# umr-lops/xsarsea

Measured on AMD Instinct MI355X. Metric: Mpixels/s wind inversion (CMOD5.N, 20k x 20k sigma0), higher is better.
Workload: dtype f64; 1 GPU; CMOD5.N mono-VV inversion (the metric's raster), 20000x20000 float32 sigma0/incidence + complex64 ancillary, default LUT 501x499x181 (90319 candidates/pixel), complex64 out, algo=pruned, sigma0 -> dB fused on the device; lines=20000, samples=20000, lines_rank0=20000, parallelism=row tiles x1

## Files before the change

xsarsea_amd/csrc/xsw_band.hpp:

```cpp
#pragma once
#include "xsw_device.hpp"

namespace xsw {

#ifndef XSW_BAND_MAX
#define XSW_BAND_MAX 64
#endif
#ifndef XSW_BAND_RAY_D
#define XSW_BAND_RAY_D 2
#endif
#ifndef XSW_LONG_RUN_MAX
#define XSW_LONG_RUN_MAX 128
#endif
#ifndef XSW_LONG_RUN_MAX_CUT
#define XSW_LONG_RUN_MAX_CUT 64
#endif
#ifndef XSW_SWEEP_MAX
#define XSW_SWEEP_MAX 128
#endif
#ifndef XSW_B2_HARD_AREA
#define XSW_B2_HARD_AREA 256
#endif
#ifndef XSW_BAND_SEEDED
#define XSW_BAND_SEEDED 1
// ... 5 lines not shown
#define XSW_BAND_WG_WAVES 4
#endif
#ifndef XSW_BAND_POOL
#define XSW_BAND_POOL 1
#endif
static_assert(XSW_BAND_WG_WAVES % 4 == 0 || !XSW_BAND_POOL, "pooled class counts are read as four bytes per word");
#ifndef XSW_BAND_WAVES
#define XSW_BAND_WAVES 8
#endif
#ifndef XSW_BAND_BATCH_S
#define XSW_BAND_BATCH_S 2
#endif
#ifndef XSW_BAND_BATCH
#define XSW_BAND_BATCH 4
#endif
#ifndef XSW_BAND_WAVES_CR
#define XSW_BAND_WAVES_CR 7
#endif
#ifndef XSW_BAND2_WAVES
#define XSW_BAND2_WAVES 4
#endif

struct BandSlot {
    double sn, thr_lo, thr_hi, ah, bh, m2;
    int inc_bin , rows , ipn ;
    int bin_hi ;
};

constexpr int kBandClasses = 11;
struct BandPool {
    alignas(4) unsigned char cnt[kBandClasses][XSW_BAND_WG_WAVES];
    unsigned short map[64 * XSW_BAND_WG_WAVES];
};
__device__ __forceinline__ int byte_sum4(unsigned x)
{
    x = (x & 0x00ff00ffu) + ((x >> 8) & 0x00ff00ffu);
    return (int)((x & 0xffffu) + (x >> 16));
}

struct BandRec {
    double s, ah, bh;
    float d;
    int inc_tail;
    int rows;
    int ipn;
    unsigned idx;
    int flags;
};
struct Band2Slot;
constexpr int kBand2SlotBytes = 56;
template <typename T, typename TO, bool CR>
// ... 41 lines not shown
            for (int e = 0; e < 2; ++e) {
                const int ip = gc + 2 * h + e;
                const int ra = (int)((wa[h] >> (e * 16)) & 0xffffu), rb = (int)((wb[h] >> (e * 16)) & 0xffffu);
                const float uh = e ? uhx * c4.z + uhy * c4.w : uhx * c4.x + uhy * c4.y;
                const int lo = max(w_lo, ra), hi = capped ? min(w_hi, rb - 1) : w_hi;
                const float t = vminf(vmaxf(uh, fmaf((float)lo, whs, wh0)), fmaf((float)max(hi, lo), whs, wh0));
                const float jw = fmaf(t, t - 2.0f * uh, m2) - XSW_BOUND_SLACK * (m2 + t * (t + 2.0f * fabsf(uh)));
                const bool live = gact && ip >= ip_lo && ip < ip_end && lo <= hi && !(jw > jub);
                first = (live && first == 0x7fff) ? ip : first;
                last = live ? ip : last;
            }
        }
    }
    return last >= 0 ? (unsigned)first | ((unsigned)last << 16) : 0x00007fffu;
}
__device__ __forceinline__ double ld_co(const char *__restrict__ base, unsigned off0, int row, unsigned rowB)
{
    return *(const double *)(base + (off0 + __umul24((unsigned)row, rowB)));
}

#ifndef XSW_CHORD_MRG
#define XSW_CHORD_MRG 2e-3
#endif
template <int S, int K, bool COUNT>
__device__ __forceinline__ void co_band_pass(const DevTables &L, double inv_dsig, int lane,
                                             const BandSlot *slots , int *res ,
                                             int first, int count , unsigned &cand,
                                             const unsigned short *map = nullptr )
{
    constexpr int sweep_max = XSW_BAND_MAX;
    const double inf = __builtin_inf();
    const int q = lane / S, sl = lane & (S - 1);
    const bool valid = q < count;
    const int owner = valid ? (map ? (int)map[first + q] : first + q) : lane;
    BandSlot B = slots[owner];
    if (!valid) { B.inc_bin = 0; B.rows = 0; B.ipn = 0; B.bin_hi = -1; }
    const int B_ip_lo = B.ipn & 0xffff, B_ncols = (int)((unsigned)B.ipn >> 16);
    const int w_lo = B.rows & 0xffff, w_hi = B.rows >> 16;
    const double thr_lo = B.thr_lo, thr_hi = B.thr_hi, sn = B.sn;
    const double wh0 = 0.5 * L.w0, whs = L.wstep_half;
    const char *__restrict__ base = (const char *)L.co;
    const unsigned rowB = (unsigned)L.phi_pad * 8u;
    const int i_inc = B.inc_bin & 0xffff;
    const unsigned slice0 = mul24_sv(rowB, mul24_sv((unsigned)L.n_w, (unsigned)i_inc));
    const unsigned short *__restrict__ inv_tab = L.inv_rows;
    const unsigned inv_rowB = (unsigned)L.phi_pad * 2u;
    const unsigned inv0 = mul24_sv(inv_rowB, (unsigned)(i_inc * XSW_INV_BINS) + ((unsigned)B.inc_bin >> 16));
    const unsigned inv1 = mul24_sv(inv_rowB, (unsigned)(i_inc * XSW_INV_BINS) + (unsigned)max(B.bin_hi, 0));
    double best = inf, second = inf;
    int brow = 0, bip = 0;
    unsigned ncand = 0;
    bool overflow = false;
    const int nchunks = S == 64 ? (__builtin_amdgcn_readfirstlane(B_ncols) + 64 * K - 1) / (64 * K) : 1;
#pragma unroll 1
    for (int ch = 0; ch < nchunks; ++ch) {
        bool act[K];
        int ip[K], r[K], nrow[K];
        unsigned off0[K];
        double U[K];
#pragma unroll
        for (int j = 0; j < K; ++j) {
            const int vcol = sl + S * j + S * K * ch;
            act[j] = valid && vcol < B_ncols;
            ip[j] = B_ip_lo + (act[j] ? vcol : 0);
            const unsigned ipB = (unsigned)ip[j] * 8u;
            const double2 cs = *(const double2 *)((const char *)L.csphi + 2u * ipB);
            U[j] = 2.0 * (B.ah * cs.x + B.bh * cs.y);
            off0[j] = slice0 + ipB;
        }
        int nmax = 0;
#pragma unroll
        for (int j = 0; j < K; ++j) {
            const unsigned o_first = inv0 + (unsigned)ip[j] * 2u, o_last = inv1 + (unsigned)ip[j] * 2u;
            const int ra = (int)*(const unsigned short *)((const char *)inv_tab + o_first);
            const int rb = (int)*(const unsigned short *)((const char *)inv_tab + o_last);
            r[j] = max(ra, w_lo);
            const int last = B.bin_hi >= 0 ? min(rb - 1, w_hi) : w_hi;
            nrow[j] = act[j] ? last - r[j] + 1 : 0;
            nmax = max(nmax, nrow[j]);
        }
#pragma unroll 1
        for (int t = 0; t < XSW_BAND_MAX; ++t) {
            unsigned long long left[K], any_left = 0ULL;
#pragma unroll
            for (int j = 0; j < K; ++j) { left[j] = ballot64(t < nrow[j]); any_left |= left[j]; }
            if (any_left == 0ULL) break;
#pragma unroll
            for (int j = 0; j < K; ++j) {
                if (left[j] == 0ULL) continue;
                const int rc = min(r[j] + t, w_hi);
                const double v = ld_co(base, off0[j], rc, rowB);
                const bool inb = t < nrow[j];
                const double wh = fma((double)rc, whs, wh0);
                const double dd = fma(v, inv_dsig, sn);
                double J = fma(dd, dd, wh * (wh - U[j]));
                J = __hiloint2double(inb ? __double2hiint(J) : 0x7FE00000, __double2loint(J));
                second = vmin(second, vmax(J, best));
                const bool lt = J < best;
                brow = lt ? rc : brow;
                if (K > 1 || S == 64) bip = lt ? ip[j] : bip;
                best = vmin(best, J);
                if (COUNT) ncand += inb ? 1u : 0u;
            }
        }
        const bool any = nmax > sweep_max;
        overflow = overflow || any;
        if (K == 1 && S != 64) bip = ip[0];
    }
    const int bflat = (int)__umul24((unsigned)brow, (unsigned)L.n_phi) + bip;
    const double gmin = S == 64 ? wave_min_d(best) : seg_min_d<S>(best);
    const double T = gmin + 1e-9 * (1.0 + fabs(gmin) + slots[owner].m2);
    const unsigned long long amb = ballot64(valid && (second <= T || overflow)), surv = ballot64(valid && best <= T);
    const unsigned long long segmask = S == 64 ? ~0ULL : (((1ULL << (S & 63)) - 1ULL) << ((q * S) & 63));
    const bool bad = (amb & segmask) != 0ULL || __popcll(surv & segmask) != 1 || !(gmin < 1e300);
    if (valid && ((!bad && best <= T) || (bad && sl == 0))) res[owner] = bad ? -1 : bflat;
    if (COUNT) {
        unsigned c = ncand;
        for (int off = 32; off > 0; off >>= 1) c += __shfl_xor(c, off);
        cand += c;
    }
}

__device__ __forceinline__ bool list_append(unsigned *__restrict__ count, unsigned *__restrict__ list, unsigned cap, bool flag, long long i, int lane)
{
    const unsigned long long um = __ballot(flag);
    if (!um) return false;
    unsigned base = 0;
    if (lane == 0) base = atomicAdd(count, (unsigned)__popcll(um));
    base = (unsigned)__builtin_amdgcn_readfirstlane((int)base);
    const unsigned at = base + __builtin_amdgcn_mbcnt_hi((unsigned)(um >> 32), __builtin_amdgcn_mbcnt_lo((unsigned)um, 0u));
    if (flag && at < cap) list[at] = (unsigned)i;
    return flag && at >= cap;
}
__device__ __forceinline__ void mask_mark(unsigned long long *__restrict__ mask, bool flag, long long i, long long strip, long long samples, int lane)
{
    const unsigned long long m = __ballot(flag);
    if (!m) return;
    if (strip >= 0) {
// ... 43 lines not shown
    if (A.list_b) drop_b = A.rec_b ? (unresolved && to_b) : list_append(A.list_b_count, A.list_b, A.list_b_cap, unresolved && to_b, i, lane);
    if (A.list_c) drop_c = list_append(A.list_c_count, A.list_c, A.list_c_cap, unresolved && to_c && !to_b, i, lane);
    const bool for_c = A.list_c != nullptr && to_c && !to_b && !drop_c;
    const bool drop_g = list_append(A.list_count, A.list, A.list_cap, unresolved && !to_b && !for_c, i, lane);
    if (A.mask_g) {
        if (A.list_b) mask_mark(A.mask_b, drop_b, i, strip, A.samples, lane);
        mask_mark(A.mask_g, drop_g, i, strip, A.samples, lane);
    }
    if (in) {
        if (!unresolved) {
            Pixel Q;
            Q.flags = flags;
            Q.a_re = nan; Q.a_im = nan;
            if (A.anc) {
                typename Cx<T>::type z = ((const typename Cx<T>::type *)A.anc)[i];
                Q.a_re = (double)z.x;
                Q.a_im = (double)z.y;
            }
            store_pixel<TO, CR>(L, A, i, Q, my_flat, my_icr);
        }
    }
}

template <typename T, typename TO, bool CR, bool COUNT, int ROLE = 0>
__device__ __forceinline__ void band_wave(const DevTables &L, const KArgs &A, long long i, bool in, int lane, BandSlot *__restrict__ slots,
                                          int *__restrict__ res_, bool strip_walk = false ,
                                          long long strip = -1 ,
                                          BandPool *__restrict__ pool = nullptr )
{
    const double nan = __builtin_nan("");
    int flags, my_flat = -1, my_icr = -1;
    unsigned cand = 0;
    constexpr int NC = kBandClasses;
    constexpr bool POOLED = XSW_BAND_POOL && ROLE != 2;
    constexpr int WG = XSW_BAND_WG_WAVES, PK = POOLED ? 64 * WG : 64;
    int pos = -1, myc = NC, first[NC] = {}, ncls[NC] = {};
    auto settle_queues = [&]() {
#pragma unroll
        for (int c = 0; c + 1 < NC; ++c) {
            const int np = 64 / (2 << (c >> 1)), npn = 64 / (2 << ((c + 1) >> 1));
            const int rem = ncls[c] % np;
            const int added = (ncls[c + 1] + rem + npn - 1) / npn - (ncls[c + 1] + npn - 1) / npn;
            if (rem > 0 && added == 0) { ncls[c] -= rem; ncls[c + 1] += rem; first[c + 1] -= rem; }
        }
#pragma unroll
        for (int c = 0; c < NC; ++c) {
            first[c] = __builtin_amdgcn_readfirstlane(first[c]);
            ncls[c] = __builtin_amdgcn_readfirstlane(ncls[c]);
        }
    };
    bool skip = false;
    {
        Pixel P;
        load_pixel<T, false>(L, A, i, in, P);
        flags = P.flags;
        if (CR && A.s_cr) {
            const T x = ((const T *)A.s_cr)[i];
            const T dr = A.dsig_cr ? ((const T *)A.dsig_cr)[i] : (T)0;
            if (x != x || dr != dr) flags |= F_CR_RAW_NAN;
        }
        const unsigned long long todo = __ballot((P.flags & F_NEED_CO) != 0);
        bool eligb = false;
        int ncols_p = 0;
        if (todo) {
            bool loose = false;
            CoWindow W = co_window_lanes<XSW_BAND_RAYS, XSW_BAND_RAY_D, XSW_BAND_SEEDED != 0>(L, P, A.inv_dsig_co, fabs(A.dsig_co), loose);
            int w_hi_e = W.w_hi;
            bool has_tail = false;
            if (L.tail_min) {
                const bool fin1 = (P.flags & F_NEED_CO) != 0 && (P.flags & F_CO_FINITE) != 0;
                const int mono1 = L.mono_rows[fin1 ? P.i_inc : 0];
                if (fin1 && W.w_hi >= mono1 && W.ip_hi >= W.ip_lo) {
                    const int len = W.ip_hi - W.ip_lo + 1, k = min(31 - __clz(len), XSW_TAIL_LEVELS);
                    const double *tk = L.tail_min + mul24_sv((unsigned)L.phi_pad, (unsigned)(P.i_inc * (XSW_TAIL_LEVELS + 1) + k));
                    const double lo = fmin(tk[W.ip_lo], tk[k < XSW_TAIL_LEVELS ? W.ip_hi - (1 << k) + 1 : W.ip_lo]);
                    if (P.s_co + W.band_d < lo) w_hi_e = mono1 - 1;
                    else if (ROLE != 0 && mono1 >= 1 && W.w_hi - mono1 + 1 <= A.tail_max) { has_tail = true; w_hi_e = mono1 - 1; }
                }
            }
            const int nrows_p = w_hi_e - W.w_lo + 1;
            ncols_p = W.ip_hi - W.ip_lo + 1;
            const bool need = (P.flags & F_NEED_CO) != 0 && (P.flags & F_CO_FINITE) != 0 && ncols_p >= 1 && (nrows_p >= 1 || has_tail);
            if (ROLE == 2 && strip_walk) skip = !need || !(w_hi_e < L.mono_rows[need ? P.i_inc : 0]);
            eligb = need && w_hi_e < L.mono_rows[need ? P.i_inc : 0];
            if (ROLE != 2 && need && !eligb) flags |= F_TO_C;
            if (COUNT) cand += (unsigned)__popcll(__ballot(eligb)) * (unsigned)(2 * (32 - __clz((L.n_w + 1) >> 1)) + (XSW_BAND_RAYS - 1) * 2 * XSW_RAY_SIDE_STEPS);
            double thr_lo = P.s_co - W.band_d, thr_hi = P.s_co + W.band_d;
            int bin = 0, bhi = XSW_INV_BINS;
            if (eligb) {
                const double *g = L.inv_grid + 3 * P.i_inc;
                const double t0 = g[0], width = g[1];
                bin = (int)fmin(fmax((thr_lo - t0) * g[2], 0.0), (double)(XSW_INV_BINS - 1));
                if (bin > 0 && fma((double)bin, width, t0) > thr_lo) --bin;
                if (bin > 0 && fma((double)bin, width, t0) > thr_lo) bin = 0;
// ... 70 lines not shown
                const unsigned long long m = __ballot(myc == c);
                const int rank = (int)__builtin_amdgcn_mbcnt_hi((unsigned)(m >> 32), __builtin_amdgcn_mbcnt_lo((unsigned)m, 0u));
                pos = myc == c ? base + rank : pos;
                first[c] = base;
                ncls[c] = __popcll(m);
                base += ncls[c];
            }
            if constexpr (!POOLED) settle_queues();
            const bool to_rec = ROLE == 1 && A.rec_b != nullptr && (flags & F_TO_B) != 0;
            if constexpr (ROLE == 2) {
                const bool mine = in && !(strip_walk && (skip || (flags & F_NEED_CO) == 0));
                BandRec r;
                r.s = P.s_co; r.ah = 0.5 * P.a_re; r.bh = 0.5 * P.b_eff; r.d = __double2float_ru(W.band_d);
                r.inc_tail = P.i_inc | ((has_tail ? W.w_hi - w_hi_e : 0) << 16);
                r.rows = W.w_lo | (w_hi_e << 16); r.ipn = W.ip_lo | (ncols_p << 16);
                r.idx = (unsigned)i; r.flags = flags | F_B2_HARD;
                band2_core<T, TO, CR>(L, A, r, mine, mine && eligb, lane, (Band2Slot *)slots, res_, strip);
                return;
            }
            BandSlot b;
            if (eligb) {
                const double ah = 0.5 * P.a_re, bh = 0.5 * P.b_eff;
                b.sn = -P.s_co * A.inv_dsig_co; b.thr_lo = thr_lo; b.thr_hi = thr_hi;
                b.ah = ah; b.bh = bh; b.m2 = ah * ah + bh * bh;
                b.inc_bin = P.i_inc | (bin << 16); b.rows = W.w_lo | (w_hi_e << 16); b.ipn = W.ip_lo | (ncols_p << 16);
                b.bin_hi = bhi < XSW_INV_BINS ? bhi : -1;
            }
            if (ROLE == 1 && A.rec_b != nullptr) {
                const unsigned long long hm = __ballot(to_rec);
                if (hm) {
                    unsigned at0 = 0;
                    if (lane == 0) at0 = atomicAdd(A.list_b_count, (unsigned)__popcll(hm));
                    at0 = (unsigned)__builtin_amdgcn_readfirstlane((int)at0);
                    const unsigned at = at0 + __builtin_amdgcn_mbcnt_hi((unsigned)(hm >> 32), __builtin_amdgcn_mbcnt_lo((unsigned)hm, 0u));
                    if (to_rec && at < A.list_b_cap) {
                        BandRec r;
                        r.s = P.s_co; r.ah = 0.5 * P.a_re; r.bh = 0.5 * P.b_eff; r.d = __double2float_ru(W.band_d);
                        r.inc_tail = P.i_inc | ((has_tail ? W.w_hi - w_hi_e : 0) << 16);
                        r.rows = W.w_lo | (w_hi_e << 16); r.ipn = W.ip_lo | (ncols_p << 16);
                        r.idx = (unsigned)i;
                        r.flags = (flags & ~F_TO_B) | (hard ? F_B2_HARD : 0);
                        ((BandRec *)A.rec_b)[at] = r;
                        flags |= F_REC_DONE;
                    }
                }
            }
            if (eligb) {
                slots[pos] = b;
#ifdef XSW_TIMING_STAGE1_ONLY
                res_[pos] = 0;
#else
                res_[pos] = -1;
#endif
            }
        }
    }
    res_[PK + lane] = pos;
    const int wv = POOLED ? __builtin_amdgcn_readfirstlane((int)(threadIdx.x >> 6)) : 0;
    if constexpr (POOLED) {
        static_assert((WG & (WG - 1)) == 0, "passes are dealt to the waves modulo XSW_BAND_WG_WAVES");
        if (lane == 0) {
#pragma unroll
            for (int c = 0; c < NC; ++c) pool->cnt[c][wv] = (unsigned char)ncls[c];
        }
        __syncthreads();
        int e = 0, base = 0;
#pragma unroll
        for (int c = 0; c < NC; ++c) {
            int n = 0, before = 0;
#pragma unroll
            for (int k = 0; k < WG / 4; ++k) {
                const unsigned x = (unsigned)__builtin_amdgcn_readfirstlane((int)((const unsigned *)pool->cnt[c])[k]);
                const int lo = wv - 4 * k;
                n += byte_sum4(x);
                before += byte_sum4(lo >= 4 ? x : lo <= 0 ? 0u : x & ((1u << (8 * lo)) - 1u));
            }
            e = myc == c ? base + before - first[c] : e;
            first[c] = base;
            ncls[c] = n;
            base += n;
        }
        settle_queues();
        if (pos >= 0) pool->map[pos + e] = (unsigned short)(wv * 64 + pos);
        __syncthreads();
    } else {
        __builtin_amdgcn_fence(__ATOMIC_RELEASE, "wavefront");
        __builtin_amdgcn_wave_barrier();
        __builtin_amdgcn_fence(__ATOMIC_ACQUIRE, "wavefront");
    }
#ifdef XSW_BAND_PASS_STATS
    unsigned long long pst[8] = {};
#endif
#ifndef XSW_TIMING_STAGE1_ONLY
    {
        int dealt = 0;
        auto run = [&](auto seg, auto kk, int c) {
            constexpr int S = decltype(seg)::value, K = decltype(kk)::value, np = 64 / S;
            if constexpr (POOLED) {
                const int npass = (ncls[c] + np - 1) / np;
                for (int p = (wv - dealt) & (WG - 1); p < npass; p += WG) {
                    co_band_pass<S, K, COUNT>(L, A.inv_dsig_co, lane, slots - 64 * wv, res_ - 64 * wv, first[c] + p * np, min(np, ncls[c] - p * np), cand,
                                              pool->map);
#ifdef XSW_BAND_PASS_STATS
                    pst[c < 7 ? c : 7] += (1ULL << 32) + (unsigned long long)min(np, ncls[c] - p * np);
#endif
                }
                dealt += npass;
            } else {
                for (int p = 0; p < ncls[c]; p += np) {
                    co_band_pass<S, K, COUNT>(L, A.inv_dsig_co, lane, slots, res_, first[c] + p, min(np, ncls[c] - p), cand);
#ifdef XSW_BAND_PASS_STATS
                    pst[c < 7 ? c : 7] += (1ULL << 32) + (unsigned long long)min(np, ncls[c] - p);
#endif
                }
            }
        };
        using two = std::integral_constant<int, 2>;
        using three = std::integral_constant<int, 3>;
#ifndef XSW_BAND_WIDE_K
#define XSW_BAND_WIDE_K three
#endif
        run(std::integral_constant<int, 2>{}, two{}, 0);
        run(std::integral_constant<int, 2>{}, three{}, 1);
        run(std::integral_constant<int, 4>{}, two{}, 2);
        run(std::integral_constant<int, 4>{}, three{}, 3);
        run(std::integral_constant<int, 8>{}, two{}, 4);
        run(std::integral_constant<int, 8>{}, three{}, 5);
        run(std::integral_constant<int, 16>{}, two{}, 6);
        run(std::integral_constant<int, 16>{}, three{}, 7);
        run(std::integral_constant<int, 32>{}, two{}, 8);
        run(std::integral_constant<int, 32>{}, three{}, 9);
        run(std::integral_constant<int, 64>{}, XSW_BAND_WIDE_K{}, 10);
    }
#endif
    if constexpr (POOLED) {
        __syncthreads();
    } else {
        __builtin_amdgcn_fence(__ATOMIC_RELEASE, "wavefront");
        __builtin_amdgcn_wave_barrier();
        __builtin_amdgcn_fence(__ATOMIC_ACQUIRE, "wavefront");
    }
#ifdef XSW_BAND_PASS_STATS
    if (A.stats && lane == 0) {
#pragma unroll
        for (int k = 0; k < 8; ++k)
            if (pst[k]) atomicAdd(&A.stats[k], pst[k]);
    }
#endif
    pos = res_[PK + lane];
    if (pos >= 0) my_flat = res_[pos];
    if (ROLE == 1 && (flags & F_REC_DONE) != 0) in = false;
    if (ROLE == 2 && strip_walk) {
        skip = skip || (flags & F_NEED_CO) == 0;
        in = in && !skip;
    }
    wave_tail<T, TO, CR, COUNT>(L, A, i, in, lane, flags, my_flat, strip, cand);
}

template <typename T, typename TO, bool CR, bool COUNT, int ROLE = 0>
__global__ __launch_bounds__(64 * XSW_BAND_WG_WAVES, CR ? XSW_BAND_WAVES_CR : XSW_BAND_WAVES) void k_invert_band(DevTables L, KArgs A)
{
    const int lane = threadIdx.x & 63, wv = threadIdx.x >> 6;
    __shared__ BandSlot slots[XSW_BAND_WG_WAVES][64];
    __shared__ int res_[XSW_BAND_WG_WAVES][128];
#if XSW_BAND_POOL
    __shared__ BandPool pool;
#endif
    const long long strips_per_line = (A.samples + 63) >> 6;
    const long long cols_per_xcd = (strips_per_line + 7) >> 3;
    const long long xcd = blockIdx.x & 7;
    const long long col = xcd * cols_per_xcd + blockIdx.y;
    const long long line = (long long)(blockIdx.x >> 3) * XSW_BAND_WG_WAVES + wv;
    const long long smp = col * 64 + lane;
#if XSW_BAND_POOL
    if (col >= strips_per_line) return;
    const bool live = line < A.lines;
    const bool in = live && smp < A.samples;
    const long long i = (live ? line : A.lines - 1) * A.samples + (smp < A.samples ? smp : A.samples - 1);
    band_wave<T, TO, CR, COUNT, ROLE>(L, A, i, in, lane, slots[wv], &res_[0][0] + 64 * wv, false, line * strips_per_line + col, &pool);
#else
    if (col >= strips_per_line || line >= A.lines) return;
    const bool in = smp < A.samples;
    const long long i = line * A.samples + (in ? smp : A.samples - 1);
    band_wave<T, TO, CR, COUNT, ROLE>(L, A, i, in, lane, slots[wv], res_[wv], false, line * strips_per_line + col);
#endif
}

}
```

xsarsea_amd/csrc/xsw_device.hpp:

```cpp
#pragma once
#include <hip/hip_runtime.h>
#include <stdint.h>

#include <type_traits>

#include "xsw_codes.hpp"
#include "xsw_lutplan.hpp"

namespace xsw {

struct DevTables {
    const double *co;
    const double *coT;
    const double *inc, *w, *wh, *phi, *cphi, *sphi;
    const double *csphi;
    const float *csphi32;
    const float *co32;
    const float *wh32;
    double co_absmax;
    const double *out_dir;
    const double *abs_co;
    const double *dual_dir;
    const double *sol;
    int n_inc, n_w, n_phi, phi_pad, w_pad;
// ... 364 lines not shown
        chunk_geom(width, max(W.w_hi - W.w_lo + 1, 1), L.co_off32 ? seg_lanes(width) : 64, W.geom, W.mdiv);
    }
    return W;
}

#ifndef XSW_STRIP_RAYS
#define XSW_STRIP_RAYS 3
#endif
#ifndef XSW_RAY_SIDE_STEPS
#define XSW_RAY_SIDE_STEPS 2
#endif
__device__ __forceinline__ double ray_probe(const double *__restrict__ ray, int mid, int n_w, double whs, double wh0, double inv_dsig,
                                            double sn, double ur, bool &right)
{
    const double2 v = *(const double2 *)(ray + 2 * mid);
    const double wh_a = fma((double)(2 * mid), whs, wh0), wh_b = wh_a + whs;
    const double da = fma(v.x, inv_dsig, sn), db = fma(v.y, inv_dsig, sn);
    const double Ja = fma(da, da, wh_a * (wh_a - ur));
    const double Jb = (2 * mid + 1 < n_w) ? fma(db, db, wh_b * (wh_b - ur)) : __builtin_inf();
    right = Jb < Ja;
    return vmin(Ja, Jb);
}
template <int NRAYS = 1, int RAY_D = 2, bool SEEDED = false>
__device__ __forceinline__ CoWindow co_window_lanes(const DevTables &L, const Pixel &P, double inv_dsig, double abs_dsig, bool &loose)
{
    const double inf = __builtin_inf();
    const bool fin = (P.flags & F_CO_FINITE) != 0;
    const double a = fin ? P.a_re : 0.0, b = fin ? P.b_eff : 0.0, s = fin ? P.s_co : 0.0;
    const double mag = fin ? P.mag : 0.0, theta = fin ? P.theta : 0.0;
    const double ah = 0.5 * a, bh = 0.5 * b, m2 = ah * ah + bh * bh, sn = -s * inv_dsig;
    const double wh0 = 0.5 * L.w0, whs = L.wstep_half;
    const int npairs = (L.n_w + 1) >> 1;
    double rbest = inf;
    int seed = 0;
#pragma unroll 1
    for (int q = 0; q < NRAYS; ++q) {
        const int dq = ((q + 1) >> 1) * RAY_D + (q > 2 ? 1 : 0);
        const int ipr = fin ? min(max(P.ipr + ((q & 1) ? -dq : dq), 0), L.n_phi - 1) : 0;
        const double2 csr = ((const double2 *)L.csphi)[ipr];
        const double ur = 2.0 * (ah * csr.x + bh * csr.y);
        const double *__restrict__ ray =
            L.band_mul24 ? (const double *)((const char *)L.coT + mul24_sv((unsigned)L.w_pad * 8u, mul24_sv((unsigned)L.n_phi, (unsigned)(fin ? P.i_inc : 0)) + (unsigned)ipr))
                         : L.coT + ((size_t)(fin ? P.i_inc : 0) * L.n_phi + ipr) * L.w_pad;
        if (SEEDED && q == 0) {
            int lo = 0, hi = fin ? npairs : 0;
            int mid = npairs >> 1;
            if (fin) {
                const double *g = L.inv_grid + 3 * P.i_inc;
                const int bin = (int)fmin(fmax((s - g[0]) * g[2], 0.0), (double)(XSW_INV_BINS - 1));
                mid = min((int)L.inv_rows[mul24_sv((unsigned)L.phi_pad, (unsigned)(P.i_inc * XSW_INV_BINS + bin)) + (unsigned)ipr] >> 1, npairs - 1);
            }
            int stride = 1, state = 0;
#pragma unroll 1
            while (__ballot(lo < hi) != 0ULL) {
                bool right;
                const double j = ray_probe(ray, mid, L.n_w, whs, wh0, inv_dsig, sn, ur, right);
                rbest = vmin(rbest, j);
                const bool open = lo < hi;
                lo = (open && right) ? mid + 1 : lo;
                hi = (open && !right) ? mid : hi;
                state = state == 0 ? (right ? 1 : 2) : ((state == 1 && right) || (state == 2 && !right)) ? state : 3;
                const int far = state == 1 ? lo + stride - 1 : hi - stride;
                mid = state == 3 ? (lo + hi) >> 1 : far;
                mid = min(max(mid, lo), max(hi - 1, 0));
                stride <<= 1;
            }
            seed = lo;
            continue;
        }
        constexpr int half = 1 << (XSW_RAY_SIDE_STEPS - 1);
        int lo = q == 0 ? 0 : max(seed - half, 0), hi = q == 0 ? npairs : min(seed + half, npairs);
        for (int it = (q == 0 ? 32 - __clz(npairs) : XSW_RAY_SIDE_STEPS); it > 0; --it) {
            const int mid = min((lo + hi) >> 1, npairs - 1);
            bool right;
            const double j = ray_probe(ray, mid, L.n_w, whs, wh0, inv_dsig, sn, ur, right);
            rbest = vmin(rbest, j);
            const bool open = lo < hi;
            lo = (open && right) ? mid + 1 : lo;
            hi = (open && !right) ? mid : hi;
// ... 577 lines not shown
template <typename TO> __device__ __forceinline__ void store_opt(void *out, long long i, double v)
{
    if (out) ((TO *)out)[i] = (TO)v;
}
template <typename T> __device__ __forceinline__ double dsig_cr_at(const void *raster, long long i, T x, double scalar)
{
    return raster ? (double)((const T *)raster)[i] : (double)(T)(x * (T)0 + (T)scalar);
}
template <typename T> __device__ __forceinline__ void anc_at(const void *anc, long long i, bool fold, double &a, double &b)
{
    const typename Cx<T>::type z = ((const typename Cx<T>::type *)anc)[i];
    a = (double)z.x;
    b = fold ? fabs((double)z.y) : (double)z.y;
}


template <typename T, bool CR = true>
__device__ __forceinline__ void load_pixel(const DevTables &L, const KArgs &A, long long il, bool in, Pixel &P)
{
    const double nan = __builtin_nan("");
    const double inc = ld<T>(A.inc, il);
    P.s_co = nan; P.s_cr = nan; P.dsig = nan; P.a_re = nan; P.a_im = nan;
    if (A.s_co) P.s_co = to_db(((const T *)A.s_co)[il], A.is_db);
    if (CR && A.s_cr) {
        const T x = ((const T *)A.s_cr)[il];
        P.s_cr = to_db(x, A.is_db);
        P.dsig = dsig_cr_at<T>(A.dsig_cr, il, x, A.dsig_cr_scalar);
    }
    if (A.anc) anc_at<T>(A.anc, il, false, P.a_re, P.a_im);
    P.flags = 0; P.i_inc = 0; P.i_inc_cr = 0;
    if (in) {
        const bool anc_nan = (P.a_re != P.a_re || P.a_im != P.a_im) && !(isinf(P.a_re) || isinf(P.a_im));
        if (inc != inc || (P.s_co == P.s_co && anc_nan)) P.flags = F_EARLY_NAN;
        else {
            if (P.s_co == P.s_co) {
                P.flags |= F_NEED_CO;
                P.i_inc = nearest_index(L.inc, L.n_inc, inc, L.inc_uniform != 0, L.inc0, L.inv_incstep);
                if (fabs(P.s_co) < 1e100 && fabs(P.a_re) < 1e100 && fabs(P.a_im) < 1e100) P.flags |= F_CO_FINITE;
            }
            if (P.s_cr == P.s_cr && P.dsig == P.dsig) {
                P.flags |= F_NEED_CR;
                P.i_inc_cr = nearest_index(L.inc_cr, L.n_inc_cr, inc, L.inc_cr_uniform != 0, L.inc_cr0, L.inv_inccrstep);
            }
        }
    }
    P.b_eff = L.phi_180 ? fabs(P.a_im) : P.a_im;
// ... 11 lines not shown
{
    const double nan = __builtin_nan("");
    double co_re, co_im, cr_re, cr_im;
    int o_iw = -1, o_ip = -1;
    int sgn = 0;
    if (P.flags & F_EARLY_NAN) {
        co_re = nan; co_im = 0.0; cr_re = nan; cr_im = 0.0;
    } else {
        if (P.flags & F_NEED_CO) {
            o_iw = (int)(((double)my_flat + 0.5) * L.inv_nphi);
            o_ip = my_flat - o_iw * L.n_phi;
            const double w = L.w[o_iw];
            const double2 e1 = ((const double2 *)L.out_dir)[o_ip];
            const double s1r = w * e1.x, s1i = w * e1.y + 0.0 * e1.x;
            co_re = s1r; co_im = s1i;
            if (L.phi_180) {
                const double2 e2 = ((const double2 *)L.out_dir)[L.n_phi + o_ip];
                const double s2r = w * e2.x, s2i = w * e2.y + 0.0 * e2.x;
                const double xs = P.a_im * e1.y, mag = fabs(P.a_re) + fabs(P.a_im);
                const bool clear = fabs(xs) > 1e-9 * mag && mag > 1e-100 && mag < 1e100 && w > 1e-100 && w < 1e100 && e2.y == -e1.y &&
                                   e2.x == e1.x;
                bool second = xs < 0.0;
                if (!clear) {
                    const double d1 = angle_of_quotient(P.a_re, P.a_im, s1r, s1i);
                    const double d2 = angle_of_quotient(P.a_re, P.a_im, s2r, s2i);
                    second = !(fabs(d1) <= fabs(d2));
                }
                if (second) { co_re = s2r; co_im = s2i; sgn = 1; }
            }
        } else {
            co_re = nan; co_im = nan;
        }
        if (P.flags & F_NEED_CR) {
            const double wd = L.wcr[my_icr];
            if (P.flags & F_NEED_CO) {
                const double2 u = ((const double2 *)L.dual_dir)[((size_t)sgn * L.n_w + o_iw) * L.n_phi + o_ip];
                cr_re = wd * u.x;
                cr_im = wd * u.y + 0.0 * u.x;
            } else {
                cr_re = wd; cr_im = 0.0;
            }
        } else {
            cr_re = nan; cr_im = nan;
        }
    }
    typedef typename Cx<TO>::type cx_t;
// ... 209 lines not shown
```

xsarsea_amd/csrc/xsw_invert_tu.hip:

```cpp
#include <hip/hip_runtime.h>

#include <algorithm>
#include <string>
#include <type_traits>

#include "xsw_host.hpp"
#include "xsw_band.hpp"
#include "xsw_band2.hpp"
#include "xsw_blocks.hpp"
#include "xsw_exhaustive.hpp"
#include "xsw_cross.hpp"
#include "xsw_cost.hpp"
#include "xsw_uncertainty.hpp"
#include "xsw_forward.hpp"
#include "xsw_solve.hpp"
#include "xsw_dirsolve.hpp"
#include "xsw_joint.hpp"
#include "xsw_uncertainty_joint.hpp"

using namespace xsw;

template <typename F>
static void with_pol(bool dual, F &&f)
{
    if (dual) f(std::true_type{});
    else f(std::false_type{});
}

template <typename T, typename TO>
static int launch_invert(xsw_ctx *c, const KArgs &A_in, int algo, const LaunchCtl &lc, std::string &err)
{
    const RouteFacts f = route_facts(c->T, A_in, algo, lc);
    const ChainPlan p(route_knobs(), f, ChainWaves{XSW_BAND_WG_WAVES, XSW_BAND2_WAVES, XSW_BLOCKS_WAVES});
    if (p.route == ChainPlan::TOO_LARGE) return seterr(err, XSW_EINVAL, "raster too large for one launch");
    if (p.route == ChainPlan::EXHAUSTIVE)
        return launch_exhaustive<T, TO>(c->T, A_in, lc.stream, algo == XSW_ALGO_EXHAUSTIVE) == hipSuccess
                   ? XSW_OK : seterr(err, XSW_EHIP, "exhaustive launch failed: %s", hipGetErrorString(hipGetLastError()));
    KArgs A = A_in;
    A.block_min = p.block_min;
    if (p.route == ChainPlan::CHAIN) {
        KArgs B = A;
        const WorkLists &wl = lc.lists;
        B.list_count = wl.count(WorkLists::G); B.list = wl.entries(WorkLists::G); B.list_cap = wl.cap(WorkLists::G);
        if (p.band2) { B.list_b_count = wl.count(WorkLists::B); B.list_b = wl.entries(WorkLists::B); B.list_b_cap = wl.cap(WorkLists::B); }
        static_assert(sizeof(BandRec) == XSW_REC_BYTES, "XSW_REC_BYTES (xsw_plan.hpp) is sizeof(BandRec)");
        B.rec_b = p.records ? wl.records() : nullptr;
        if (p.blocks3) { B.list_c_count = wl.count(WorkLists::C); B.list_c = wl.entries(WorkLists::C); B.list_c_cap = wl.cap(WorkLists::C); }
        B.long_run = p.long_run; B.area_max = p.area_max; B.b2_crowd = p.b2_crowd; B.area_crowd_max = p.area_crowd_max;
        B.wide_min = p.wide_min; B.arc_min = p.arc_min; B.arc_crowd = p.arc_crowd; B.b2_refine_min = p.b2_refine_min;
        B.b2_rows_max = p.b2_rows_max; B.tail_max = p.tail_max;
        if (p.masks) {
            B.mask_g = wl.masks(); B.mask_b = wl.masks() + p.nstrips;
            if (hipMemsetAsync(wl.masks(), 0, 2 * p.nstrips * sizeof(unsigned long long), lc.stream) != hipSuccess) return seterr(err, XSW_EHIP, "strip-mask reset failed");
        }
        if (hipMemsetAsync(wl.count(WorkLists::G), 0, 3 * sizeof(unsigned), lc.stream) != hipSuccess) return seterr(err, XSW_EHIP, "work-list reset failed");
        const dim3 band_grid(p.band_grid_x, p.band_grid_y), band_block(64 * XSW_BAND_WG_WAVES);
        with_pol(!f.mono, [&](auto cr) {
            constexpr bool CR = decltype(cr)::value;
            if (lc.timing) timing_mark(c);
            if (p.count_inst) hipLaunchKernelGGL((k_invert_band<T, TO, CR, true>), band_grid, band_block, 0, lc.stream, c->T, B);
            else if (p.band2) hipLaunchKernelGGL((k_invert_band<T, TO, CR, false, 1>), band_grid, band_block, 0, lc.stream, c->T, B);
            else hipLaunchKernelGGL((k_invert_band<T, TO, CR, false>), band_grid, band_block, 0, lc.stream, c->T, B);
            if (lc.timing) timing_mark(c);
#ifdef XSW_BAND_PASS_STATS
            B.stats = nullptr;
#endif
            if (p.band2) hipLaunchKernelGGL((k_invert_band2<T, TO, CR>), dim3(p.band2_blocks), band_block, 0, lc.stream, c->T, B);
            if (lc.timing) timing_mark(c);
            if (p.blocks3) hipLaunchKernelGGL((k_invert_blocks<T, TO, CR>), dim3(p.blocks3_blocks), dim3(256), 0, lc.stream, c->T, B);
            if (lc.timing) timing_mark(c);
            hipLaunchKernelGGL((k_invert_list<T, TO, CR>), dim3(p.list_blocks), dim3(256), 0, lc.stream, c->T, B);
            if (lc.timing) timing_mark(c);
        });
    } else if (p.route == ChainPlan::ONE_PRUNED) {
        with_pol(!f.mono, [&](auto cr) {
            hipLaunchKernelGGL((k_invert<T, TO, 1, decltype(cr)::value>), dim3((unsigned)p.nblocks), dim3(256), 0, lc.stream, c->T, A);
        });
    } else {
        hipLaunchKernelGGL((k_invert<T, TO, 3>), dim3((unsigned)p.nblocks), dim3(256), 0, lc.stream, c->T, A);
    }
    const hipError_t e = hipGetLastError();
    if (e != hipSuccess) return seterr(err, XSW_EHIP, "launch failed: %s", hipGetErrorString(e));
    return XSW_OK;
}


#ifndef XSW_PAIR
// ... 21 lines not shown
```

xsarsea_amd/csrc/xsw_plan.hpp:

```cpp
#pragma once
#include <algorithm>
#include <climits>
#include <cstddef>
#include <cstdlib>

#ifndef XSW_LIST_B_SHARE
#define XSW_LIST_B_SHARE 4
#endif
#ifndef XSW_LIST_C_SHARE
#define XSW_LIST_C_SHARE 4
#endif
#define XSW_LISTS_TOTAL (1 + XSW_LIST_B_SHARE + XSW_LIST_C_SHARE)
#define XSW_REC_BYTES 48

static inline size_t pad256(size_t b) { return (b + 255) & ~(size_t)255; }

struct WorkLists {
    enum List { G = 0, B = 1, C = 2 };
    unsigned *base = nullptr;
    size_t list_cap = 0;
    size_t mask_strips = 0;

    static size_t share(List l) { return l == G ? 1 : l == B ? XSW_LIST_B_SHARE : XSW_LIST_C_SHARE; }
    static size_t lists_bytes(size_t cap) { return pad256((XSW_LISTS_TOTAL * cap + 16) * sizeof(unsigned)); }
// ... 148 lines not shown
        k.no_strip_masks = env_flag("XSW_NO_STRIP_MASKS");
        k.list_cap_test = env_int("XSW_LIST_CAP_TEST", 0, 16);
        k.fail_list_alloc = env_flag("XSW_FAIL_LIST_ALLOC");
        return k;
    }
};

struct RouteFacts {
    enum Algo { PRUNED = 1, EXHAUSTIVE = 2, EXACT = 3, EXHAUSTIVE_F64 = 4 };
    bool prunable, co_off32, band_mul24, cr_monotone, blk_span_ok;
    bool mono_rows, inv_rows, blk, csphi32, tail_min;
    int n_w, n_phi;
    long long lines, samples, n;
    int algo;
    bool s_co, s_cr;
    bool mono;
    bool stats, stats_chain;
    bool lists;
    size_t mask_strips;
};

struct ChainWaves {
    int band_wg, band2, blocks;
};

struct ChainPlan {
    enum Route { EXHAUSTIVE, CHAIN, ONE_PRUNED, ONE_EXACT, TOO_LARGE };
    enum Limit { NONE, NBLOCKS, BAND_GROUPS, BAND_COLS };
    Route route;
    Limit limit = NONE;
    long long nblocks;
    int block_min;
    bool count_inst = false;
    bool band2 = false;
    bool records = false;
    bool blocks3 = false;
    bool masks = false;
    size_t nstrips = 0;
    int long_run = 0, area_max = 0, b2_crowd = 0, area_crowd_max = 0, wide_min = 0, arc_min = 0, arc_crowd = 0, b2_refine_min = 0,
        b2_rows_max = 0, tail_max = 0;
    unsigned band_grid_x = 0, band_grid_y = 0, band2_blocks = 0, blocks3_blocks = 0, list_blocks = 0;

    ChainPlan(const RouteKnobs &k, const RouteFacts &f, const ChainWaves &w) : block_min(k.block_min)
    {
        const long long strips_per_line = (f.samples + 63) / 64, line_groups = (f.lines + 3) / 4;
        nblocks = 8 * ((strips_per_line + 7) / 8) * line_groups;
        if (nblocks > 0x7fffffffLL) { route = TOO_LARGE; limit = NBLOCKS; return; }
        if (f.algo == RouteFacts::EXHAUSTIVE || f.algo == RouteFacts::EXHAUSTIVE_F64) { route = EXHAUSTIVE; return; }
        if (!(f.algo == RouteFacts::PRUNED && !k.no_band && f.lists && f.s_co && f.prunable && f.mono_rows && f.inv_rows && f.co_off32 &&
              f.band_mul24 && (!f.s_cr || f.cr_monotone) && f.n < (1LL << 32))) {
            route = f.algo == RouteFacts::PRUNED ? ONE_PRUNED : ONE_EXACT;
            return;
        }
        const long long cols_per_xcd = (strips_per_line + 7) / 8;
        const long long band_groups = (f.lines + w.band_wg - 1) / w.band_wg;
        if (8 * band_groups > 0x7fffffffLL) { route = TOO_LARGE; limit = BAND_GROUPS; return; }
        if (cols_per_xcd > 65535) { route = TOO_LARGE; limit = BAND_COLS; return; }
        route = CHAIN;
        count_inst = f.stats && !f.stats_chain;
        band2 = k.long_run > 0 && !count_inst;
        records = band2 && !k.no_records;
        blocks3 = f.blk && f.blk_span_ok && !k.no_blocks_kernel && f.n_w < 32768 && f.n_phi < 32768;
        long_run = k.long_run;
        area_max = f.blk ? k.b2_area : 0x7fffffff;
        b2_crowd = k.b2_crowd;
        area_crowd_max = 1 << 20;
        wide_min = k.b2_wide > 0 ? k.b2_wide : 0x7fffffff;
        arc_min = (k.arc_min > 0 && f.csphi32) ? k.arc_min : 0x7fffffff;
        arc_crowd = k.arc_crowd;
        b2_refine_min = k.b2_refine_min;
        b2_rows_max = k.b2_rows_max;
        tail_max = (band2 && f.tail_min) ? k.tail_sweep : 0;
        nstrips = (size_t)(strips_per_line * f.lines);
        masks = nstrips <= f.mask_strips && !k.no_strip_masks;
        band_grid_x = (unsigned)(8 * band_groups);
        band_grid_y = (unsigned)cols_per_xcd;
        band2_blocks = (unsigned)std::min<long long>(nblocks, 256 * w.band2);
        blocks3_blocks = (unsigned)std::min<long long>(nblocks, 256 * w.blocks);
        list_blocks = (unsigned)std::min<long long>(nblocks, 256 * 8);
    }
};
```

Before: 10920 Mpixels/s.

## Stage direction table in LDS and pack band results into slot records

When the phi count fits a cap (181 <= 192 here), the pooled band kernel copies the cos/sin direction table into LDS once per workgroup, published by the existing barrier, so co_band_pass reads it from LDS instead of global memory. The separate per-wave res_ LDS array is removed: results and positions now live inside BandSlot. The m2 field is dropped and recomputed from ah/bh through a volatile LDS reload. This cuts LDS footprint and global loads, possibly improving occupancy, at the cost of extra LDS traffic and code complexity. It also adds detour-counting stats compiled only under a debug macro, plus a profiling script.

```diff
diff --git a/profiles/band_detours.py b/profiles/band_detours.py
--- /dev/null
+++ b/profiles/band_detours.py
@@ -0,0 +1,44 @@
+#!/usr/bin/env python3
+import json
+import os
+import sys
+
+import torch
+
+REPO = os.path.dirname(os.path.dirname(os.path.abspath(__file__)))
+sys.path.insert(0, REPO)
+import bench
+from xsarsea_amd import _lib
+
+lines = samples = int(os.environ.get("XSW_TRAFFIC_N", "20000"))
+dev = torch.device("cuda", 0)
+lut, co = bench.build_product_lut()
+ctx = _lib.Context(0)
+ctx.upload_luts(co=co)
+inc, s_vv, anc = bench.make_scene(lines, samples, lines, 0, 20260322, dev)
+out = torch.empty((lines, samples), dtype=torch.complex64, device=dev)
+torch.cuda.synchronize()
+ctx.stats_enable(2)
+ctx.invert_raw(lines, samples, _lib.XSW_F32, _lib.XSW_F32, _lib.MEM_DEVICE, inc.data_ptr(), s_vv.data_ptr(), None, None,
+               anc.data_ptr(), out.data_ptr(), None, algo=_lib.ALGO_PRUNED)
+st, ch = ctx.stats(), ctx.stats_chain()
+ctx.stats_enable(False)
+all_waves = lines * ((samples + 63) // 64)
+waves = st["pixels_co"]
+if not 0 < waves <= all_waves:
+    sys.exit("not a -DXSW_BAND_DETOUR_STATS build: slot 0 holds %d, the raster has %d waves" % (waves, all_waves))
+res = {
+    "what": "k_invert_band detour counters (-DXSW_BAND_DETOUR_STATS, production chain, headline scene %d^2 CMOD5.N mono float32); per wave" % lines,
+    "waves": all_waves,
+    "waves_with_co_search": waves,
+    "nan_sigma0_share": float(torch.isnan(s_vv).float().mean()),
+    "log10_detour_waves": st["cand_co"], "log10_detour_share": st["cand_co"] / all_waves,
+    "store_near_tie_waves": st["pixels_exact"], "store_near_tie_share": st["pixels_exact"] / all_waves,
+    "tail_cut_branch_waves": st["pixels_cr"], "tail_cut_branch_share": st["pixels_cr"] / all_waves,
+    "first_ray_trips": ch["cand_band2"], "first_ray_trips_per_wave": ch["cand_band2"] / waves,
+}
+print(json.dumps(res, indent=1))
+if len(sys.argv) > 1:
+    with open(sys.argv[1], "w") as f:
+        json.dump(res, f, indent=1)
+        f.write("\n")
diff --git a/xsarsea_amd/csrc/xsw_band.hpp b/xsarsea_amd/csrc/xsw_band.hpp
--- a/xsarsea_amd/csrc/xsw_band.hpp
+++ b/xsarsea_amd/csrc/xsw_band.hpp
@@ -51,11 +51,16 @@
 #endif
 
 struct BandSlot {
-    double sn, thr_lo, thr_hi, ah, bh, m2;
+    double sn, thr_lo, thr_hi, ah, bh;
+    int res, pos;
     int inc_bin , rows , ipn ;
     int bin_hi ;
 };
 
+#ifndef XSW_BAND_CS_CAP
+#define XSW_BAND_CS_CAP 192
+#endif
+constexpr int kBandCsCap = XSW_BAND_CS_CAP;
 constexpr int kBandClasses = 11;
 struct BandPool {
     alignas(4) unsigned char cnt[kBandClasses][XSW_BAND_WG_WAVES];
@@ -143,11 +148,12 @@
 #ifndef XSW_CHORD_MRG
 #define XSW_CHORD_MRG 2e-3
 #endif
-template <int S, int K, bool COUNT>
+template <int S, int K, bool COUNT, bool PACKED = false, bool CSLDS = false>
 __device__ __forceinline__ void co_band_pass(const DevTables &L, double inv_dsig, int lane,
-                                             const BandSlot *slots , int *res ,
+                                             BandSlot *slots , int *res ,
                                              int first, int count , unsigned &cand,
-                                             const unsigned short *map = nullptr )
+                                             const unsigned short *map = nullptr ,
+                                             const double2 *cs_lds = nullptr )
 {
     constexpr int sweep_max = XSW_BAND_MAX;
     const double inf = __builtin_inf();
@@ -185,7 +191,9 @@
             act[j] = valid && vcol < B_ncols;
             ip[j] = B_ip_lo + (act[j] ? vcol : 0);
             const unsigned ipB = (unsigned)ip[j] * 8u;
-            const double2 cs = *(const double2 *)((const char *)L.csphi + 2u * ipB);
+            double2 cs;
+            if constexpr (CSLDS) cs = cs_lds[ip[j]];
+            else cs = *(const double2 *)((const char *)L.csphi + 2u * ipB);
             U[j] = 2.0 * (B.ah * cs.x + B.bh * cs.y);
             off0[j] = slice0 + ipB;
         }
@@ -230,11 +238,17 @@
     }
     const int bflat = (int)__umul24((unsigned)brow, (unsigned)L.n_phi) + bip;
     const double gmin = S == 64 ? wave_min_d(best) : seg_min_d<S>(best);
-    const double T = gmin + 1e-9 * (1.0 + fabs(gmin) + slots[owner].m2);
+    const volatile __attribute__((address_space(3))) BandSlot *again = (const volatile __attribute__((address_space(3))) BandSlot *)(slots + owner);
+    const double ah_t = again->ah, bh_t = again->bh;
+    const double ah2 = ah_t * ah_t, bh2 = bh_t * bh_t;
+    const double T = gmin + 1e-9 * (1.0 + fabs(gmin) + (ah2 + bh2));
     const unsigned long long amb = ballot64(valid && (second <= T || overflow)), surv = ballot64(valid && best <= T);
     const unsigned long long segmask = S == 64 ? ~0ULL : (((1ULL << (S & 63)) - 1ULL) << ((q * S) & 63));
     const bool bad = (amb & segmask) != 0ULL || __popcll(surv & segmask) != 1 || !(gmin < 1e300);
-    if (valid && ((!bad && best <= T) || (bad && sl == 0))) res[owner] = bad ? -1 : bflat;
+    if (valid && ((!bad && best <= T) || (bad && sl == 0))) {
+        if constexpr (PACKED) slots[owner].res = bad ? -1 : bflat;
+        else res[owner] = bad ? -1 : bflat;
+    }
     if (COUNT) {
         unsigned c = ncand;
         for (int off = 32; off > 0; off >>= 1) c += __shfl_xor(c, off);
@@ -324,11 +338,13 @@
     }
 }
 
-template <typename T, typename TO, bool CR, bool COUNT, int ROLE = 0>
+template <typename T, typename TO, bool CR, bool COUNT, int ROLE = 0, bool CSLDS = false>
 __device__ __forceinline__ void band_wave(const DevTables &L, const KArgs &A, long long i, bool in, int lane, BandSlot *__restrict__ slots,
-                                          int *__restrict__ res_, bool strip_walk = false ,
+                                          int *__restrict__ res_ ,
+                                          bool strip_walk = false ,
                                           long long strip = -1 ,
-                                          BandPool *__restrict__ pool = nullptr )
+                                          BandPool *__restrict__ pool = nullptr ,
+                                          double2 *cs_lds = nullptr )
 {
     const double nan = __builtin_nan("");
     int flags, my_flat = -1, my_icr = -1;
@@ -336,6 +352,9 @@
     constexpr int NC = kBandClasses;
     constexpr bool POOLED = XSW_BAND_POOL && ROLE != 2;
     constexpr int WG = XSW_BAND_WG_WAVES, PK = POOLED ? 64 * WG : 64;
+    const long long i_first = POOLED ? (long long)(((unsigned long long)(unsigned)__builtin_amdgcn_readfirstlane((int)((unsigned long long)i >> 32)) << 32) |
+                                                   (unsigned)__builtin_amdgcn_readfirstlane((int)(unsigned)i)) : 0;
+    int i_delta = POOLED ? (int)(i - i_first) : 0;
     int pos = -1, myc = NC, first[NC] = {}, ncls[NC] = {};
     auto settle_queues = [&]() {
 #pragma unroll
@@ -366,12 +385,25 @@
         int ncols_p = 0;
         if (todo) {
             bool loose = false;
+#ifdef XSW_BAND_DETOUR_STATS
+            unsigned ray_trips = 0;
+            CoWindow W = co_window_lanes<XSW_BAND_RAYS, XSW_BAND_RAY_D, XSW_BAND_SEEDED != 0>(L, P, A.inv_dsig_co, fabs(A.dsig_co), loose, &ray_trips);
+            if (ROLE != 2 && A.stats && A.stats_chain && lane == 0) {
+                atomicAdd(&A.stats[0], 1ULL);
+                atomicAdd(&A.stats[4], (unsigned long long)ray_trips);
+            }
+#else
             CoWindow W = co_window_lanes<XSW_BAND_RAYS, XSW_BAND_RAY_D, XSW_BAND_SEEDED != 0>(L, P, A.inv_dsig_co, fabs(A.dsig_co), loose);
+#endif
             int w_hi_e = W.w_hi;
             bool has_tail = false;
             if (L.tail_min) {
                 const bool fin1 = (P.flags & F_NEED_CO) != 0 && (P.flags & F_CO_FINITE) != 0;
                 const int mono1 = L.mono_rows[fin1 ? P.i_inc : 0];
+#ifdef XSW_BAND_DETOUR_STATS
+                if (ROLE != 2 && A.stats && A.stats_chain && __ballot(fin1 && W.w_hi >= mono1 && W.ip_hi >= W.ip_lo) != 0ULL && lane == 0)
+                    atomicAdd(&A.stats[3], 1ULL);
+#endif
                 if (fin1 && W.w_hi >= mono1 && W.ip_hi >= W.ip_lo) {
                     const int len = W.ip_hi - W.ip_lo + 1, k = min(31 - __clz(len), XSW_TAIL_LEVELS);
                     const double *tk = L.tail_min + mul24_sv((unsigned)L.phi_pad, (unsigned)(P.i_inc * (XSW_TAIL_LEVELS + 1) + k));
@@ -488,7 +520,7 @@
             if (eligb) {
                 const double ah = 0.5 * P.a_re, bh = 0.5 * P.b_eff;
                 b.sn = -P.s_co * A.inv_dsig_co; b.thr_lo = thr_lo; b.thr_hi = thr_hi;
-                b.ah = ah; b.bh = bh; b.m2 = ah * ah + bh * bh;
+                b.ah = ah; b.bh = bh;
                 b.inc_bin = P.i_inc | (bin << 16); b.rows = W.w_lo | (w_hi_e << 16); b.ipn = W.ip_lo | (ncols_p << 16);
                 b.bin_hi = bhi < XSW_INV_BINS ? bhi : -1;
             }
@@ -512,22 +544,33 @@
                 }
             }
             if (eligb) {
-                slots[pos] = b;
 #ifdef XSW_TIMING_STAGE1_ONLY
-                res_[pos] = 0;
+                b.res = 0;
 #else
-                res_[pos] = -1;
-#endif
-            }
-        }
-    }
-    res_[PK + lane] = pos;
+                b.res = -1;
+#endif
+                BandSlot &d = slots[pos];
+                d.sn = b.sn; d.thr_lo = b.thr_lo; d.thr_hi = b.thr_hi; d.ah = b.ah; d.bh = b.bh;
+                d.inc_bin = b.inc_bin; d.rows = b.rows; d.ipn = b.ipn; d.bin_hi = b.bin_hi;
+                if constexpr (POOLED) d.res = b.res;
+                else res_[pos] = b.res;
+            }
+        }
+    }
+    if constexpr (POOLED) slots[lane].pos = pos;
+    else res_[PK + lane] = pos;
     const int wv = POOLED ? __builtin_amdgcn_readfirstlane((int)(threadIdx.x >> 6)) : 0;
     if constexpr (POOLED) {
         static_assert((WG & (WG - 1)) == 0, "passes are dealt to the waves modulo XSW_BAND_WG_WAVES");
         if (lane == 0) {
 #pragma unroll
             for (int c = 0; c < NC; ++c) pool->cnt[c][wv] = (unsigned char)ncls[c];
+        }
+        double2 cs_in;
+        const bool cs_mine = CSLDS && (int)threadIdx.x < L.n_phi;
+        if constexpr (CSLDS) {
+            static_assert(kBandCsCap <= 64 * WG, "one table entry per thread");
+            if (cs_mine) cs_in = ((const double2 *)L.csphi)[threadIdx.x];
         }
         __syncthreads();
         int e = 0, base = 0;
@@ -548,6 +591,9 @@
         }
         settle_queues();
         if (pos >= 0) pool->map[pos + e] = (unsigned short)(wv * 64 + pos);
+        if constexpr (CSLDS) {
+            if (cs_mine) cs_lds[threadIdx.x] = cs_in;
+        }
         __syncthreads();
     } else {
         __builtin_amdgcn_fence(__ATOMIC_RELEASE, "wavefront");
@@ -565,8 +611,8 @@
             if constexpr (POOLED) {
                 const int npass = (ncls[c] + np - 1) / np;
                 for (int p = (wv - dealt) & (WG - 1); p < npass; p += WG) {
-                    co_band_pass<S, K, COUNT>(L, A.inv_dsig_co, lane, slots - 64 * wv, res_ - 64 * wv, first[c] + p * np, min(np, ncls[c] - p * np), cand,
-                                              pool->map);
+                    co_band_pass<S, K, COUNT, true, CSLDS>(L, A.inv_dsig_co, lane, slots - 64 * wv, nullptr, first[c] + p * np, min(np, ncls[c] - p * np), cand,
+                                                           pool->map, cs_lds);
 #ifdef XSW_BAND_PASS_STATS
                     pst[c < 7 ? c : 7] += (1ULL << 32) + (unsigned long long)min(np, ncls[c] - p * np);
 #endif
@@ -613,8 +659,15 @@
             if (pst[k]) atomicAdd(&A.stats[k], pst[k]);
     }
 #endif
-    pos = res_[PK + lane];
-    if (pos >= 0) my_flat = res_[pos];
+    if constexpr (POOLED) {
+        __asm__ volatile("" : "+v"(i_delta));
+        i = i_first + i_delta;
+        pos = slots[lane].pos;
+        if (pos >= 0) my_flat = slots[pos].res;
+    } else {
+        pos = res_[PK + lane];
+        if (pos >= 0) my_flat = res_[pos];
+    }
     if (ROLE == 1 && (flags & F_REC_DONE) != 0) in = false;
     if (ROLE == 2 && strip_walk) {
         skip = skip || (flags & F_NEED_CO) == 0;
@@ -623,14 +676,17 @@
     wave_tail<T, TO, CR, COUNT>(L, A, i, in, lane, flags, my_flat, strip, cand);
 }
 
-template <typename T, typename TO, bool CR, bool COUNT, int ROLE = 0>
+template <typename T, typename TO, bool CR, bool COUNT, int ROLE = 0, bool CSLDS = false>
 __global__ __launch_bounds__(64 * XSW_BAND_WG_WAVES, CR ? XSW_BAND_WAVES_CR : XSW_BAND_WAVES) void k_invert_band(DevTables L, KArgs A)
 {
+    static_assert(!CSLDS || XSW_BAND_POOL, "the LDS copy of the direction table is published by the pooled queues' barriers");
     const int lane = threadIdx.x & 63, wv = threadIdx.x >> 6;
     __shared__ BandSlot slots[XSW_BAND_WG_WAVES][64];
-    __shared__ int res_[XSW_BAND_WG_WAVES][128];
 #if XSW_BAND_POOL
     __shared__ BandPool pool;
+    __shared__ double2 cs_lds[CSLDS ? kBandCsCap : 1];
+#else
+    __shared__ int res_[XSW_BAND_WG_WAVES][128];
 #endif
     const long long strips_per_line = (A.samples + 63) >> 6;
     const long long cols_per_xcd = (strips_per_line + 7) >> 3;
@@ -643,7 +699,7 @@
     const bool live = line < A.lines;
     const bool in = live && smp < A.samples;
     const long long i = (live ? line : A.lines - 1) * A.samples + (smp < A.samples ? smp : A.samples - 1);
-    band_wave<T, TO, CR, COUNT, ROLE>(L, A, i, in, lane, slots[wv], &res_[0][0] + 64 * wv, false, line * strips_per_line + col, &pool);
+    band_wave<T, TO, CR, COUNT, ROLE, CSLDS>(L, A, i, in, lane, slots[wv], nullptr, false, line * strips_per_line + col, &pool, cs_lds);
 #else
     if (col >= strips_per_line || line >= A.lines) return;
     const bool in = smp < A.samples;
diff --git a/xsarsea_amd/csrc/xsw_device.hpp b/xsarsea_amd/csrc/xsw_device.hpp
--- a/xsarsea_amd/csrc/xsw_device.hpp
+++ b/xsarsea_amd/csrc/xsw_device.hpp
@@ -410,7 +410,11 @@
     return vmin(Ja, Jb);
 }
 template <int NRAYS = 1, int RAY_D = 2, bool SEEDED = false>
-__device__ __forceinline__ CoWindow co_window_lanes(const DevTables &L, const Pixel &P, double inv_dsig, double abs_dsig, bool &loose)
+__device__ __forceinline__ CoWindow co_window_lanes(const DevTables &L, const Pixel &P, double inv_dsig, double abs_dsig, bool &loose
+#ifdef XSW_BAND_DETOUR_STATS
+                                                    , unsigned *first_ray_trips = nullptr
+#endif
+)
 {
     const double inf = __builtin_inf();
     const bool fin = (P.flags & F_CO_FINITE) != 0;
@@ -443,6 +447,9 @@
             while (__ballot(lo < hi) != 0ULL) {
                 bool right;
                 const double j = ray_probe(ray, mid, L.n_w, whs, wh0, inv_dsig, sn, ur, right);
+#ifdef XSW_BAND_DETOUR_STATS
+                if (first_ray_trips) ++*first_ray_trips;
+#endif
                 rbest = vmin(rbest, j);
                 const bool open = lo < hi;
                 lo = (open && right) ? mid + 1 : lo;
@@ -1066,6 +1073,12 @@
     const double inc = ld<T>(A.inc, il);
     P.s_co = nan; P.s_cr = nan; P.dsig = nan; P.a_re = nan; P.a_im = nan;
     if (A.s_co) P.s_co = to_db(((const T *)A.s_co)[il], A.is_db);
+#ifdef XSW_BAND_DETOUR_STATS
+    if (sizeof(T) == 4 && A.stats && A.stats_chain && A.s_co && !A.is_db) {
+        const float y = (float)((const T *)A.s_co)[il] + 1e-15f;
+        if (__ballot(!(y > 0.0f && y <= 3.40282347e38f)) != 0ULL && (threadIdx.x & 63) == 0) atomicAdd(&A.stats[1], 1ULL);
+    }
+#endif
     if (CR && A.s_cr) {
         const T x = ((const T *)A.s_cr)[il];
         P.s_cr = to_db(x, A.is_db);
@@ -1123,6 +1136,12 @@
                                    e2.x == e1.x;
                 bool second = xs < 0.0;
                 if (!clear) {
+#ifdef XSW_BAND_DETOUR_STATS
+                    if (A.stats && A.stats_chain) {
+                        const unsigned long long m = __ballot(true);
+                        if ((int)(threadIdx.x & 63) == __ffsll((long long)m) - 1) atomicAdd(&A.stats[2], 1ULL);
+                    }
+#endif
                     const double d1 = angle_of_quotient(P.a_re, P.a_im, s1r, s1i);
                     const double d2 = angle_of_quotient(P.a_re, P.a_im, s2r, s2i);
                     second = !(fabs(d1) <= fabs(d2));
diff --git a/xsarsea_amd/csrc/xsw_invert_tu.hip b/xsarsea_amd/csrc/xsw_invert_tu.hip
--- a/xsarsea_amd/csrc/xsw_invert_tu.hip
+++ b/xsarsea_amd/csrc/xsw_invert_tu.hip
@@ -31,7 +31,7 @@
 static int launch_invert(xsw_ctx *c, const KArgs &A_in, int algo, const LaunchCtl &lc, std::string &err)
 {
     const RouteFacts f = route_facts(c->T, A_in, algo, lc);
-    const ChainPlan p(route_knobs(), f, ChainWaves{XSW_BAND_WG_WAVES, XSW_BAND2_WAVES, XSW_BLOCKS_WAVES});
+    const ChainPlan p(route_knobs(), f, ChainWaves{XSW_BAND_WG_WAVES, XSW_BAND2_WAVES, XSW_BLOCKS_WAVES, XSW_BAND_POOL ? kBandCsCap : 0});
     if (p.route == ChainPlan::TOO_LARGE) return seterr(err, XSW_EINVAL, "raster too large for one launch");
     if (p.route == ChainPlan::EXHAUSTIVE)
         return launch_exhaustive<T, TO>(c->T, A_in, lc.stream, algo == XSW_ALGO_EXHAUSTIVE) == hipSuccess
@@ -58,11 +58,19 @@
         with_pol(!f.mono, [&](auto cr) {
             constexpr bool CR = decltype(cr)::value;
             if (lc.timing) timing_mark(c);
-            if (p.count_inst) hipLaunchKernelGGL((k_invert_band<T, TO, CR, true>), band_grid, band_block, 0, lc.stream, c->T, B);
-            else if (p.band2) hipLaunchKernelGGL((k_invert_band<T, TO, CR, false, 1>), band_grid, band_block, 0, lc.stream, c->T, B);
-            else hipLaunchKernelGGL((k_invert_band<T, TO, CR, false>), band_grid, band_block, 0, lc.stream, c->T, B);
+            auto band = [&](auto lds) {
+                constexpr bool CSLDS = decltype(lds)::value;
+                if (p.count_inst) hipLaunchKernelGGL((k_invert_band<T, TO, CR, true, 0, CSLDS>), band_grid, band_block, 0, lc.stream, c->T, B);
+                else if (p.band2) hipLaunchKernelGGL((k_invert_band<T, TO, CR, false, 1, CSLDS>), band_grid, band_block, 0, lc.stream, c->T, B);
+                else hipLaunchKernelGGL((k_invert_band<T, TO, CR, false, 0, CSLDS>), band_grid, band_block, 0, lc.stream, c->T, B);
+            };
+#if XSW_BAND_POOL
+            if (p.cs_lds) band(std::true_type{});
+            else
+#endif
+                band(std::false_type{});
             if (lc.timing) timing_mark(c);
-#ifdef XSW_BAND_PASS_STATS
+#if defined(XSW_BAND_PASS_STATS) || defined(XSW_BAND_DETOUR_STATS)
             B.stats = nullptr;
 #endif
             if (p.band2) hipLaunchKernelGGL((k_invert_band2<T, TO, CR>), dim3(p.band2_blocks), band_block, 0, lc.stream, c->T, B);
diff --git a/xsarsea_amd/csrc/xsw_plan.hpp b/xsarsea_amd/csrc/xsw_plan.hpp
--- a/xsarsea_amd/csrc/xsw_plan.hpp
+++ b/xsarsea_amd/csrc/xsw_plan.hpp
@@ -194,6 +194,7 @@
 
 struct ChainWaves {
     int band_wg, band2, blocks;
+    int band_cs_cap = 0;
 };
 
 struct ChainPlan {
@@ -207,6 +208,7 @@
     bool band2 = false;
     bool records = false;
     bool blocks3 = false;
+    bool cs_lds = false;
     bool masks = false;
     size_t nstrips = 0;
     int long_run = 0, area_max = 0, b2_crowd = 0, area_crowd_max = 0, wide_min = 0, arc_min = 0, arc_crowd = 0, b2_refine_min = 0,
@@ -232,6 +234,7 @@
         count_inst = f.stats && !f.stats_chain;
         band2 = k.long_run > 0 && !count_inst;
         records = band2 && !k.no_records;
+        cs_lds = f.n_phi >= 1 && f.n_phi <= w.band_cs_cap;
         blocks3 = f.blk && f.blk_span_ok && !k.no_blocks_kernel && f.n_w < 32768 && f.n_phi < 32768;
         long_run = k.long_run;
         area_max = f.blk ? k.b2_area : 0x7fffffff;
```

After: 11210 Mpixels/s, median of 6. +2.6%, better.
